# willi-menapace/PlayableVideoGeneration

Hardware: AMD Instinct MI355X
Metric: training clips/sec (B x16x256x256) (higher is better)
Workload: dtype f32; 1 GPU; bair256_t16_b8; variant=main, per_gpu_batch=8, global_batch=8, seq_len=16, gt_init=6, parallelism=dp1

## Files before the change

### include/caddy_hip.h

```cpp
#ifndef CADDY_HIP_H
#define CADDY_HIP_H
#include <stddef.h>
#ifdef __cplusplus
extern "C" {
#endif

typedef struct caddy_ctx caddy_ctx;

typedef struct caddy_config {
    int variant;
    int batch;
    int seq_len;
    int height, width;
    int stacking;
    int actions;
    int action_dim;
    int hidden;
    int use_gumbel, hard_gumbel, use_variations;
    float centroid_alpha;
    int perceptual;
    int ensemble;
} caddy_config;
#define CADDY_MAX_ENSEMBLE 8

// ... 74 lines not shown
int caddy_set_grads_ready_hook(caddy_ctx* ctx, caddy_grads_ready_hook hook, void* user);
int caddy_dp_available(void);
int caddy_dp_unique_id(char* out256);
int caddy_dp_init(caddy_ctx* ctx, const char* id256, int world_size, int rank, int overlap);
int caddy_allreduce_grads(caddy_ctx* ctx);
long caddy_dp_bucket_floats(caddy_ctx* ctx);
int caddy_dp_shutdown(caddy_ctx* ctx);
typedef void (*caddy_sampler_hook)(const float* log_probs, const float* sampled_dirs, float* samples, float* variations,
                                   int n, int K, int Da, int stage, void* user);
int caddy_set_sampler_hook(caddy_ctx* ctx, caddy_sampler_hook hook, void* user, int provides_samples, int provides_variations);
int caddy_set_allreduce_hook(caddy_ctx* ctx, void (*hook)(float* device_ptr, int count, void* user), void* user, int world_size);

int caddy_forward_full(caddy_ctx* ctx, const float* obs, int gt_init, float tau, const caddy_noise* noise, int training,
                       const float* samples_in, const float* variations_in);
int caddy_forward_pretraining(caddy_ctx* ctx, const float* obs, float tau, const caddy_noise* noise, int training,
                              const float* samples_in, const float* variations_in);
int caddy_get_output(caddy_ctx* ctx, int id, void* dst);
int caddy_get_output_grad(caddy_ctx* ctx, int id, void* dst);

int caddy_loss_backward(caddy_ctx* ctx, const caddy_loss_cfg* cfg, double* losses_host);

int caddy_adam_step(caddy_ctx* ctx, float* m, float* v, float lr, float beta1, float beta2, float eps, float weight_decay,
                    int step, float grad_scale);
int caddy_set_action_member(caddy_ctx* ctx, int member);
int caddy_adam_step_member(caddy_ctx* ctx, float* m, float* v, float lr, float beta1, float beta2, float eps, float weight_decay, int step, int member_step, float grad_scale);
int caddy_adam_step_ex(caddy_ctx* ctx, float* m, float* v, float lr, float beta1, float beta2, float eps, float weight_decay, int step, const int* member_step, int s2h_step,
                       float grad_scale);

int caddy_start_inference(caddy_ctx* ctx);
int caddy_f16_saturated(caddy_ctx* ctx);
int caddy_fallback_layers(caddy_ctx* ctx);
int caddy_generate_next(caddy_ctx* ctx, const float* observation, int action, const float* variation, float* frame_out, float* obs_out);

#define CADDY_PROFILE_FAMILIES 18
int caddy_debug_set_poison(caddy_ctx* ctx, int on);
int caddy_debug_set_seeds_only(caddy_ctx* ctx, int on);
int caddy_profile_begin(caddy_ctx* ctx);
int caddy_profile_end(caddy_ctx* ctx, double* out );
int caddy_profile_records(caddy_ctx* ctx, double* out, int max_records);
int caddy_profile_phases(caddy_ctx* ctx, char* names_out, float* ms_out, int max);

int caddy_debug_count(caddy_ctx* ctx);
int caddy_debug_fusion_counts(caddy_ctx* ctx, long* out3);
int caddy_debug_set_bn_paths(caddy_ctx* ctx, int small, int lazy, int epilogue_stats);
int caddy_debug_set_vgg_s16(caddy_ctx* ctx, int on);
int caddy_debug_set_s16_grads(caddy_ctx* ctx, int on);
int caddy_debug_set_perc_chunks(caddy_ctx* ctx, int n);
long caddy_debug_s16_grad_count(caddy_ctx* ctx);
int caddy_debug_set_pack_merged(caddy_ctx* ctx, int on);
int caddy_debug_dims(caddy_ctx* ctx, int i, int* nhwc4);
int caddy_debug_get(caddy_ctx* ctx, int i, int grad, float* dst_nchw);

int caddy_bn_layer_count(caddy_ctx* ctx);
long caddy_bn_calls(caddy_ctx* ctx, int i, char* name_out128);

struct ConvArgs; struct WgradArgs; struct PackDesc; struct TV;
int caddy_k_conv_fwd(const struct ConvArgs* a, void* stream);
int caddy_k_conv_wgrad(const struct WgradArgs* a, void* stream);
int caddy_k_conv_took_direct(void);
int caddy_k_conv_stats_tiles(void);
int caddy_k_bn_finalize_tiles(const float* part, int ntiles, int ldp, long count, const float* gamma, const float* beta, float* rmean, float* rvar, int C,
                              float* mean, float* invstd, float* scale, float* shift, void* stream);
int caddy_k_bn_bwd_lazy(const struct TV* dout, const struct TV* x, const float* mean, const float* invstd, const float* gamma, const float* scale, const float* shift, int act,
                        double* sums, double* scratch, const struct TV* dx, float* dgamma, float* dbeta, void* stream);
int caddy_k_conv_pick_bn(int cout);
int caddy_k_hx_pick_bn(int cout);
int caddy_k_hx_force_big(int v);
// ... 13 lines not shown
```

### playablevideogeneration_amd/csrc/build.py

```python
import os
import subprocess
import sys

HERE = os.path.dirname(os.path.abspath(__file__))
ROOT = os.path.dirname(os.path.dirname(HERE))
SOURCES = ["conv_mfma.hip", "conv_hx.hip", "conv_hx_wgrad.hip", "conv_head.hip", "conv_direct.hip", "conv_thin.hip", "conv_narrow.hip", "conv_stream.hip", "pointwise.hip", "pack.hip", "head.hip", "perceptual.hip", "frame_metrics.hip", "lpips.hip", "detection.hip", "net.cpp", "capi_kernels.cpp", "dp_rccl.cpp"]
LIB = os.path.join(HERE, "libcaddy_hip.so")


def _stale(target, deps):
    if not os.path.exists(target):
        return True
    t = os.path.getmtime(target)
    return any(os.path.getmtime(d) > t for d in deps)


def _deps():
    return [os.path.join(HERE, f) for f in os.listdir(HERE) if f.endswith((".hip", ".cpp", ".h"))] + \
           [os.path.join(ROOT, "include", "caddy_hip.h")]


def _compile_objects(cmd_prefix, objdir, srcs, headers):
    os.makedirs(objdir, exist_ok=True)
    objs, procs = [], []
    for src in srcs:
        obj = os.path.join(objdir, os.path.basename(src) + ".o")
        objs.append(obj)
        if _stale(obj, [src] + headers):
            procs.append((src, subprocess.Popen(cmd_prefix + ["-c", src, "-o", obj])))
    for src, p in procs:
        if p.wait() != 0:
            raise RuntimeError("compile failed: " + src)
    return objs


def build(force=False):
    srcs = [os.path.join(HERE, s) for s in SOURCES if os.path.exists(os.path.join(HERE, s))]
    headers = [d for d in _deps() if d.endswith(".h")]
    if not force and not _stale(LIB, _deps()):
# ... 12 lines not shown
```

### playablevideogeneration_amd/csrc/capi_kernels.cpp

```cpp
#include "common.h"
#include "pointwise.h"
#include "pack.h"

#define ST(s) ((hipStream_t)(s))
extern "C" {
int caddy_k_conv_fwd(const ConvArgs* a, void* s) { return conv_fwd_launch(*a, ST(s)); }
int caddy_k_conv_took_direct(void) { return g_last_conv_direct; }
int caddy_k_conv_stats_tiles(void) { return g_last_conv_stats_tiles; }
int caddy_k_bn_finalize_tiles(const float* part, int ntiles, int ldp, long count, const float* gamma, const float* beta, float* rmean, float* rvar, int C,
                              float* mean, float* invstd, float* scale, float* shift, void* s) {
    return pw_bn_finalize_tiles(part, ntiles, ldp, count, gamma, beta, rmean, rvar, C, mean, invstd, scale, shift, ST(s));
}
int caddy_k_bn_bwd_lazy(const TV* dout, const TV* x, const float* mean, const float* invstd, const float* gamma, const float* scale, const float* shift, int act,
                        double* sums, double* scratch, const TV* dx, float* dgamma, float* dbeta, void* s) {
    int rc = pw_bn_bwd_reduce(*dout, nullptr, *x, mean, invstd, sums, scratch, dgamma, dbeta, ST(s), act ? scale : nullptr, shift);
    return rc ? rc : pw_bn_bwd_apply(*dout, nullptr, *x, mean, invstd, gamma, sums, *dx, nullptr, nullptr, 1, ST(s), act ? scale : nullptr, shift);
}
int caddy_k_conv_wgrad(const WgradArgs* a, void* s) { return conv_wgrad_launch(*a, ST(s)); }
int caddy_k_conv_pick_bn(int cout) { return conv_pick_bn(cout); }
int caddy_k_conv_avgpool_ok(const ConvArgs* a) { return conv_avgpool_ok(*a); }
int caddy_k_hx_pick_bn(int cout) { return hx_pick_bn(cout); }
int caddy_k_hx_force_big(int v) { g_hx_big_override = v; return 0; }
int caddy_k_hx_set_bg(int mask) { g_hx_bg = mask; return 0; }
long caddy_k_hx_weight_bytes(const PackDesc* d, int seg, int rows_pad, int planes) { return (long)hx_weight_bytes(*d, seg, rows_pad, planes); }
int caddy_k_pack_hx(const PackDesc* d, void* wq, int rows_pad, int seg, int precision, void* s) { return pack_hx(*d, wq, rows_pad, seg, precision, ST(s)); }
int caddy_k_pack_fwd(const PackDesc* d, float* wp, void* s) { return pack_fwd(*d, wp, ST(s)); }
int caddy_k_pack_dgrad(const PackDesc* d, int seg, float* wpd, int Cd_pad, int Kd, void* s) { return pack_dgrad(*d, seg, wpd, Cd_pad, Kd, ST(s)); }
int caddy_k_unpack_wgrad(const PackDesc* d, const float* dwp, void* s) { return unpack_wgrad(*d, dwp, ST(s)); }
int caddy_k_adam(float* p, const float* g, float* m, float* v, long n, float lr, float b1, float b2, float eps, float wd, int step, float gscale, void* s) {
    return adam_launch(p, g, m, v, n, lr, b1, b2, eps, wd, step, gscale, ST(s));
}
int caddy_k_copy(const TV* a, const TV* b, int acc, void* s) { return pw_copy(*a, *b, acc, ST(s)); }
int caddy_k_pool2(const TV* in, const TV* out, void* s) { return pw_pool2(*in, *out, ST(s)); }
int caddy_k_pool2_bwd(const TV* dout, const TV* din, void* s) { return pw_pool2_bwd(*dout, *din, 0, ST(s)); }
int caddy_k_up2(const TV* in, const TV* out, void* s) { return pw_up2(*in, *out, ST(s)); }
int caddy_k_up2_bwd(const TV* dout, const TV* din, void* s) { return pw_up2_bwd(*dout, *din, ST(s)); }
int caddy_k_stats(const TV* x, double* sums, void* s) { return pw_stats(*x, sums, nullptr, ST(s)); }
int caddy_k_stats_partials(const TV* x, double* sums, double* scratch, void* s) { return pw_stats(*x, sums, scratch, ST(s)); }
int caddy_k_bn_finalize(const double* sums, long count, const float* gamma, const float* beta, float* rmean, float* rvar, int C, int training,
                        float* mean, float* invstd, float* scale, float* shift, void* s) {
// ... 50 lines not shown
```

### playablevideogeneration_amd/csrc/common.h

```cpp
#pragma once
#include <hip/hip_runtime.h>
#include <cstdint>

typedef float f32x16 __attribute__((ext_vector_type(16)));
typedef float f32x4 __attribute__((ext_vector_type(4)));
typedef __bf16 bf16x8 __attribute__((ext_vector_type(8)));
typedef __bf16 bf16x4 __attribute__((ext_vector_type(4)));

struct TV {
    float* p;
    int N, H, W, C;
    long sn;
    int ld;
    int s16;
};

static inline int cdiv(long a, long b) { return (int)((a + b - 1) / b); }
static inline int round_up(int a, int b) { return (a + b - 1) / b * b; }

#define CONV_MAX_SRC 3
#define CONV_BK 16
struct ConvSrc {
    const float* p;
    long sn;
// ... 60 lines not shown
extern thread_local int g_last_conv_lstm_fused;
#define HX_WSCALE 64.0f
enum { PREC_FP32 = 0, PREC_F16X3 = 16, PREC_BF16X3 = 17, PREC_F16X1 = 18, PREC_BF16X1 = 19 };
#define HX_KC 32
constexpr int CONV_AUX_BYTES = 128 * 1024;

struct WgradArgs {
    ConvSrc src[CONV_MAX_SRC];
    int nsrc;
    int N, H, W;
    int KS;
    const float* dy;
    long dy_sn;
    int dy_ld;
    int Cout, Cout_pad;
    int Ktot;
    float* dwp;
    int slabs;
    int group_n;
    long src_gs[CONV_MAX_SRC];
    long dy_gs;
    int precision;
    long src_bn_gs[CONV_MAX_SRC];
    float* det_slab;
    long det_cap;
    long det_stride;
    int dy_s16;
};
#define WGRAD_DST(a_, split_) ((a_).det_slab ? (a_).det_slab + (long)(split_) * (a_).det_stride : (a_).dwp)
long wgrad_det_begin(WgradArgs& a, long splits, hipStream_t st);
int wgrad_det_end(const WgradArgs& a, long splits, hipStream_t st);

enum { CK_FWD_128x128 = 0, CK_FWD_128x64, CK_FWD_64x64, CK_FWD_128x32, CK_THIN_OUT, CK_THIN_IN, CK_WGRAD_128, CK_WGRAD_64, CK_WGRAD_32, CK_WGRAD_SMALL, CK_WGRAD_THIN, CK_WGRAD_TILE, CK_NARROW,
       CK_HX_128, CK_HX_64, CK_HX_32, CK_WGRAD_HX, CK_HX_128_8W, CK_COUNT };
extern thread_local int g_last_conv_kernel;
static inline long conv_stats_tiles_cap(int N, int H, int W) { long t = (long)N * cdiv(H, 8) * cdiv(W, 16); return t > 512 ? t : 512; }
extern thread_local int g_last_conv_stats_tiles;
extern thread_local int g_last_conv_direct;
bool conv_src_lazy_ok(const ConvArgs& a);
bool wgrad_src_lazy_ok(const WgradArgs& a);
int conv_fwd_launch(const ConvArgs& a, hipStream_t st);
int conv_wgrad_launch(const WgradArgs& a, hipStream_t st);
int conv_pick_bn(int cout);
struct PackDesc;
int conv_hx_wgrad_try(const WgradArgs& a, hipStream_t st, bool dry = false);
int conv_hx_try(const ConvArgs& a, hipStream_t st, bool dry = false);
bool conv_hx_s16_ok(int N, int H, int W, int Cout);
bool conv_hx_pool_ok(int N, int H, int W, int Cout);
int pack_hx(const PackDesc& d, void* wq, int rows_pad, int seg , int precision, hipStream_t st);
size_t hx_weight_bytes(const PackDesc& d, int seg, int rows_pad, int planes);
int hx_kq(const PackDesc& d, int seg);
int hx_pick_bn(int cout);
template <int NPL> __host__ __device__ __forceinline__ long hx_wq_piece(int row, int g) { return ((long)((row >> 5) * 2 + (g >> 1)) * NPL) * 64 + (g & 1) * 32 + (row & 31); }
extern int g_hx_big_override;
extern int g_hx_bg;
int conv_split_reduce_pool_launch(const float* scr, long stride, int splits, int ldc, int N, int H, int W, int C, float* out, long out_sn, int out_ld, const float* bias, int act,
                                  const float* res, long res_sn, int res_ld, hipStream_t st);
int conv_split_reduce_lstm_launch(const float* scr, long stride, int splits, int ldc, int HW, long P, const float* bias, const LstmFuse& f, hipStream_t st);
int conv_split_reduce_launch(const float* scr, long stride, int splits, int ldc, int HW, long P, int C, float* out, long out_sn, int out_ld, const float* bias, int act,
                             const float* res, long res_sn, int res_ld, hipStream_t st, float* stats = nullptr, int stats_ld = 0, long stats_cap_tiles = 0, int accumulate = 0);
int conv_thin_fwd_try(const ConvArgs& a, hipStream_t st);
int conv_head_fwd_try(const ConvArgs& a, hipStream_t st);
int conv_head_dgrad_try(const ConvArgs& a, hipStream_t st);
int conv_hx_avgpool_ok(const ConvArgs& a);
int conv1x1_lat_try(const ConvArgs& a, hipStream_t st, bool dry = false);
int conv_direct_try(const ConvArgs& a, hipStream_t st, bool dry = false);
int conv_stream_wgrad_try(const WgradArgs& a, hipStream_t st, bool dry = false);
int conv_head_wgrad_try(const WgradArgs& a, hipStream_t st, bool dry = false);
extern thread_local int g_last_wgrad_grouped;
int conv_narrow_wgrad_try(const WgradArgs& a, hipStream_t st, bool dry = false);
int conv_c4_wgrad_try(const WgradArgs& a, hipStream_t st, bool dry = false);
int conv_c4_fwd_try(const ConvArgs& a, hipStream_t st);
int conv_narrow_fwd_try(const ConvArgs& a, hipStream_t st);
int conv_narrow_fwd_ok(const ConvArgs& a);
int conv_thin_wgrad_try(const WgradArgs& a, hipStream_t st, bool dry = false);
```

### playablevideogeneration_amd/csrc/conv_mfma.hip

```cpp
#include "common.h"
#include <cstdlib>

namespace {

constexpr int BK = CONV_BK;
constexpr int LDSK = BK + 4;

struct SegRef { const float* p; long sn; int ld; int C; int bcast; int c0; int idx; };

__device__ __forceinline__ SegRef find_seg(const ConvSrc* src, int nsrc, int k) {
    int s = 0;
    while (s + 1 < nsrc && k >= src[s].Cpad) { k -= src[s].Cpad; s++; }
    SegRef r; r.p = src[s].p; r.sn = src[s].sn; r.ld = src[s].ld; r.C = src[s].C; r.bcast = src[s].bcast; r.c0 = k; r.idx = s;
    return r;
}

__device__ __forceinline__ float4 load4_masked(const float* q, int c, int C) {
    float4 v = make_float4(0.f, 0.f, 0.f, 0.f);
    if (c + 4 <= C) v = *reinterpret_cast<const float4*>(q);
    else {
        if (c < C) v.x = q[0];
        if (c + 1 < C) v.y = q[1];
        if (c + 2 < C) v.z = q[2];
    }
// ... 857 lines not shown
    const long blocks = cdiv(a.det_stride, 256);
    hipLaunchKernelGGL(k_wgrad_det_reduce, dim3((unsigned)(blocks > 2048 ? 2048 : blocks)), dim3(256), 0, st, a.dwp, (const float*)a.det_slab, (int)splits, a.det_stride);
    return 0;
}

static int conv_wgrad_launch1(const WgradArgs& a0, hipStream_t st, bool dry);
int conv_wgrad_launch(const WgradArgs& a0, hipStream_t st) {
    if (a0.group_n <= 0 || a0.N <= a0.group_n) return conv_wgrad_launch1(a0, st, false);
    if (conv_wgrad_launch1(a0, st, true) == 0 && (g_last_conv_kernel == CK_WGRAD_TILE || g_last_conv_kernel == CK_WGRAD_HX || g_last_wgrad_grouped)) return conv_wgrad_launch1(a0, st, false);
    for (int g = 0; g * a0.group_n < a0.N; g++) {
        WgradArgs a = a0;
        a.N = a0.group_n; a.group_n = 0;
        for (int s = 0; s < a0.nsrc; s++) a.src[s].p = a0.src[s].p + g * a0.src_gs[s];
        a.dy = a0.dy + g * a0.dy_gs;
        int rc = conv_wgrad_launch1(a, st, false);
        if (rc) return rc;
    }
    return 0;
}
static int conv_wgrad_launch1(const WgradArgs& a0, hipStream_t st, bool dry) {
    WgradArgs a = a0;
    if (a.nsrc < 1 || a.nsrc > CONV_MAX_SRC) return -1;
    int bn = conv_pick_bn(a.Cout);
    if (a.Cout_pad != round_up(a.Cout, bn)) return -1;
    if (a.group_n > 0 && a.N <= a.group_n) a.group_n = 0;
    if (conv_hx_wgrad_try(a, st, dry) == 1) return 0;
    if (a.dy_s16) return -1;
    for (int s = 0; s < a.nsrc; s++) if (a.src[s].bn_scale) return -1;
    g_last_wgrad_grouped = 0;
    { int rc = conv_stream_wgrad_try(a, st, dry); if (rc != 0) return rc < 0 ? rc : 0; }
    { int rc = conv_head_wgrad_try(a, st, dry); if (rc != 0) return rc < 0 ? rc : 0; }
    if (conv_c4_wgrad_try(a, st, dry) == 1) return 0;
    if (conv_thin_wgrad_try(a, st, dry) == 1) return 0;
    if (conv_narrow_wgrad_try(a, st, dry) == 1) return 0;
    long P = (long)a.N * a.H * a.W;
    int taps = a.KS * a.KS;
    if (a.nsrc == 1 && !a.src[0].bcast && a.Cout <= 32 && a.Ktot <= 64 && a.KS <= 3 && P >= 4096 && !(a.Ktot > 32 && a.KS == 3)) {
        int tx = cdiv(a.W, STW), ty = cdiv(a.H, STH);
        long ntiles = (long)a.N * tx * ty;
        int grid = (int)(ntiles < 512 ? ntiles : 512);
        g_last_conv_kernel = CK_WGRAD_SMALL;
        if (dry) return 0;
        if (a.det_slab) { grid = (int)wgrad_det_begin(a, grid, st); if (grid <= 0) return -1; }
        if (a.Ktot <= 32) hipLaunchKernelGGL((k_conv_wgrad_small<1>), dim3(grid), dim3(256), 0, st, a, tx, ty);
        else hipLaunchKernelGGL((k_conv_wgrad_small<2>), dim3(grid), dim3(256), 0, st, a, tx, ty);
        if (a.det_slab) wgrad_det_end(a, grid, st);
        g_last_conv_kernel = CK_WGRAD_SMALL;
        return 0;
    }
    if (a.KS == 3 && a.W >= 8 && a.H >= 2) {
        int tx = cdiv(a.W, WT_W), ty = cdiv(a.H, WT_H);
        long ntiles = (long)a.N * tx * ty;
        int kt = cdiv(a.Ktot, WT_KC);
        bool o32 = a.Cout <= 32;
        int ot = o32 ? 1 : cdiv(a.Cout, 64);
        const int tile_blocks = 256;
        long g = tile_blocks / ((long)kt * ot);
        if (g < 1) g = 1;
        if (g > ntiles) g = ntiles;
        g_last_conv_kernel = CK_WGRAD_TILE;
        if (dry) return 0;
        if (a.det_slab) { g = wgrad_det_begin(a, g, st); if (g <= 0) return -1; }
        dim3 grid(kt, ot, (unsigned)g);
        if (o32) hipLaunchKernelGGL((k_conv_wgrad_tile<1>), grid, dim3(256), 0, st, a, tx, ty);
        else hipLaunchKernelGGL((k_conv_wgrad_tile<2>), grid, dim3(256), 0, st, a, tx, ty);
        if (a.det_slab) wgrad_det_end(a, g, st);
        g_last_conv_kernel = CK_WGRAD_TILE;
// ... 26 lines not shown
```

### playablevideogeneration_amd/csrc/conv_narrow.hip

```cpp
#include "common.h"
#include <cstdlib>

namespace {
constexpr int NTW = 32, NTH = 8, NHW = NTW + 2, NHH = NTH + 2;
typedef float f32x4 __attribute__((ext_vector_type(4)));

__device__ __forceinline__ float4 nld4(const float* q, int c, int C) {
    float4 v = make_float4(0.f, 0.f, 0.f, 0.f);
    if (c + 4 <= C) v = *reinterpret_cast<const float4*>(q);
    else { if (c < C) v.x = q[0]; if (c + 1 < C) v.y = q[1]; if (c + 2 < C) v.z = q[2]; }
    return v;
}

template <int CI4, int NT>
__global__ __launch_bounds__(256) void k_conv_narrow(ConvArgs a, int tiles_x, int tiles_y) {
    constexpr int CI = 16 * CI4, PITCH = CI + 4, Q = CI / 4;
    constexpr int NLOAD = (NHH * NHW * Q + 255) / 256;
    __shared__ float xs[NHH * NHW * PITCH];
    const int tid = threadIdx.x, lane = tid & 63, wave = tid >> 6;
    const int lp = lane & 15, g = lane >> 4;
    const ConvSrc s = a.src[0];
    const long ntiles = (long)a.N * tiles_x * tiles_y;

    float4 w[9][NT][CI4];
// ... 117 lines not shown

static bool narrow_shape_ok(const ConvArgs& a) {
    if (a.nsrc != 1 || a.src[0].bcast || a.src[0].bn_scale || a.KS != 3 || (a.act != 0 && a.act != 3) || a.splitk > 1) return false;
    if (a.Ktot > 32 || a.Cout > 32 || a.src[0].C <= 4 || a.Cout <= 4) return false;
    if (a.src[0].C <= 12 && a.Cout < 16) return false;
    if ((a.src[0].ld & 3) || (a.src[0].sn & 3) || a.Cout_pad < 16 * ((a.Cout + 15) / 16)) return false;
    if (a.mask || a.pool_out || a.skip_out || a.in_s16 || a.out_s16) return false;
    if ((long)a.N * a.H * a.W < 4096) return false;
    if (a.avgpool && ((a.H | a.W) & 1)) return false;
    return true;
}
int conv_narrow_fwd_ok(const ConvArgs& a) { return narrow_shape_ok(a) ? 1 : 0; }
int conv_avgpool_ok(const ConvArgs& a) {
    if (a.wq && a.precision >= PREC_F16X3) return conv_hx_avgpool_ok(a);
    ConvArgs b = a; b.avgpool = 1; b.splitk = 1;
    if (a.KS == 1) return conv1x1_lat_try(b, nullptr, true);
    return narrow_shape_ok(b) ? 1 : 0;
}

int conv_narrow_fwd_try(const ConvArgs& a, hipStream_t st) {
    if (!narrow_shape_ok(a) || (a.out_ld & 3) || (a.out_sn & 3)) return 0;
    const int tx = cdiv(a.W, NTW), ty = cdiv(a.H, NTH);
    const long ntiles = (long)a.N * tx * ty;
    const int grid = (int)(ntiles < 1024 ? ntiles : 1024);
    const int ci4 = a.Ktot / 16, nt = (a.Cout + 15) / 16;
    if (ci4 == 1 && nt == 1) hipLaunchKernelGGL((k_conv_narrow<1, 1>), dim3(grid), dim3(256), 0, st, a, tx, ty);
    else if (ci4 == 1) hipLaunchKernelGGL((k_conv_narrow<1, 2>), dim3(grid), dim3(256), 0, st, a, tx, ty);
    else if (nt == 1) hipLaunchKernelGGL((k_conv_narrow<2, 1>), dim3(grid), dim3(256), 0, st, a, tx, ty);
    else hipLaunchKernelGGL((k_conv_narrow<2, 2>), dim3(grid), dim3(256), 0, st, a, tx, ty);
    g_last_conv_kernel = CK_NARROW;
    return 1;
}

namespace {
template <int CI16, int CO16>
__global__ __launch_bounds__(256) void k_wgrad_narrow(WgradArgs a, int tiles_x, int tiles_y) {
    constexpr int PX = CI16 == 1 ? 16 : 48, PY = CO16 == 1 ? 16 : 48;
    constexpr int QX = 4 * CI16, QY = 4 * CO16;
    constexpr int NX = (NHH * NHW * QX + 255) / 256, NY = NTH * NTW * QY / 256;
    __shared__ float xs[NHH * NHW * PX];
    __shared__ float ys[NTH * NTW * PY];
    const int tid = threadIdx.x, lane = tid & 63, wave = tid >> 6;
    const int lp = lane & 15, g = lane >> 4;
    const ConvSrc s = a.src[0];
    const long ntiles = (long)a.N * tiles_x * tiles_y;
    f32x4 acc[9][CO16][CI16];
#pragma unroll
    for (int t = 0; t < 9; t++)
#pragma unroll
        for (int m = 0; m < CO16; m++)
#pragma unroll
            for (int n = 0; n < CI16; n++) acc[t][m][n] = f32x4{0.f, 0.f, 0.f, 0.f};

    float4 px[NX], py[NY];
    auto gload = [&](long tile) {
        int n = (int)(tile / (tiles_x * tiles_y));
        int rem = (int)(tile - (long)n * tiles_x * tiles_y);
        int ty = rem / tiles_x;
        int y0 = ty * NTH, x0 = (rem - ty * tiles_x) * NTW;
        const float* bx = s.p + (long)n * s.sn;
        const float* by = a.dy + (long)n * a.dy_sn;
#pragma unroll
        for (int i = 0; i < NX; i++) {
            int idx = tid + 256 * i, hp = idx / QX, c = (idx % QX) * 4;
            int hy = hp / NHW, hx = hp - hy * NHW;
            int y = y0 - 1 + hy, x = x0 - 1 + hx;
            px[i] = make_float4(0.f, 0.f, 0.f, 0.f);
            if (hp < NHH * NHW && y >= 0 && y < a.H && x >= 0 && x < a.W && c < s.C) px[i] = nld4(bx + ((long)y * a.W + x) * s.ld + c, c, s.C);
        }
#pragma unroll
        for (int i = 0; i < NY; i++) {
            int idx = tid + 256 * i, p = idx / QY, c = (idx % QY) * 4;
            int y = y0 + p / NTW, x = x0 + (p & (NTW - 1));
            py[i] = make_float4(0.f, 0.f, 0.f, 0.f);
            if (y < a.H && x < a.W && c < a.Cout) py[i] = nld4(by + ((long)y * a.W + x) * a.dy_ld + c, c, a.Cout);
        }
    };

    long tile = blockIdx.x;
    if (tile < ntiles) gload(tile);
    for (; tile < ntiles; tile += gridDim.x) {
#pragma unroll
        for (int i = 0; i < NX; i++) {
            int idx = tid + 256 * i, hp = idx / QX;
            if (hp < NHH * NHW) *reinterpret_cast<float4*>(&xs[hp * PX + (idx % QX) * 4]) = px[i];
        }
#pragma unroll
        for (int i = 0; i < NY; i++) {
            int idx = tid + 256 * i;
            *reinterpret_cast<float4*>(&ys[(idx / QY) * PY + (idx % QY) * 4]) = py[i];
        }
        __syncthreads();
        if (tile + gridDim.x < ntiles) gload(tile + gridDim.x);
#pragma unroll 2
        for (int grp = 0; grp < 16; grp++) {
            const int row = 2 * wave + (grp >> 3), x0 = 4 * (grp & 7) + g;
            float fa[CO16];
#pragma unroll
            for (int m = 0; m < CO16; m++) fa[m] = ys[(row * NTW + x0) * PY + m * 16 + lp];
#pragma unroll
            for (int t = 0; t < 9; t++) {
                const int dy = t / 3, dx = t - 3 * dy;
                const float* xp = &xs[((row + dy) * NHW + x0 + dx) * PX + lp];
#pragma unroll
                for (int n = 0; n < CI16; n++) {
                    const float fb = xp[n * 16];
#pragma unroll
                    for (int m = 0; m < CO16; m++) acc[t][m][n] = __builtin_amdgcn_mfma_f32_16x16x4f32(fa[m], fb, acc[t][m][n], 0, 0, 0);
                }
            }
        }
        __syncthreads();
    }
    constexpr int NW = 9 * CO16 * 16 * CI16 * 16;
    static_assert(NW <= NHH * NHW * PX, "LDS reduction buffer must fit in the X tile");
    float* red = xs;
    for (int i = tid; i < NW; i += 256) red[i] = 0.f;
    __syncthreads();
    for (int wv = 0; wv < 4; wv++) {
        if (wave == wv) {
#pragma unroll
            for (int t = 0; t < 9; t++)
#pragma unroll
                for (int m = 0; m < CO16; m++)
#pragma unroll
                    for (int n = 0; n < CI16; n++)
#pragma unroll
                        for (int r = 0; r < 4; r++) red[((t * CO16 * 16) + m * 16 + 4 * g + r) * (CI16 * 16) + n * 16 + lp] += acc[t][m][n][r];
        }
        __syncthreads();
    }
    float* const dst = WGRAD_DST(a, blockIdx.x);
    for (int i = tid; i < NW; i += 256) {
        int k = i % (CI16 * 16), to = i / (CI16 * 16);
        int o = to % (CO16 * 16), t = to / (CO16 * 16);
        if (k < a.Ktot && o < a.Cout) atomicAdd(dst + ((long)t * a.Cout_pad + o) * a.Ktot + k, red[i]);
    }
}
}

int conv_narrow_wgrad_try(const WgradArgs& a, hipStream_t st, bool dry) {
    if (a.nsrc != 1 || a.src[0].bcast || a.KS != 3) return 0;
    if (a.Ktot > 32 || a.Cout > 32 || a.src[0].C <= 12 || a.Cout <= 4) return 0;
    const int ci = a.Ktot / 16, co = (a.Cout + 15) / 16;
    if (ci == 2 && co == 2) return 0;
    if ((a.src[0].ld & 3) || (a.src[0].sn & 3) || (a.dy_ld & 3) || (a.dy_sn & 3)) return 0;
    if ((long)a.N * a.H * a.W < 4096) return 0;
    const int tx = cdiv(a.W, NTW), ty = cdiv(a.H, NTH);
    const long ntiles = (long)a.N * tx * ty;
    long want = ntiles / 4;
    const int grid = (int)(want < 64 ? (ntiles < 64 ? ntiles : 64) : (want < 512 ? want : 512));
    g_last_conv_kernel = CK_WGRAD_SMALL;
    if (dry) return 1;
    WgradArgs b = a;
    int gridn = grid;
    if (b.det_slab) { gridn = (int)wgrad_det_begin(b, grid, st); if (gridn <= 0) return -1; }
    if (ci == 1 && co == 1) hipLaunchKernelGGL((k_wgrad_narrow<1, 1>), dim3(gridn), dim3(256), 0, st, b, tx, ty);
    else if (ci == 1) hipLaunchKernelGGL((k_wgrad_narrow<1, 2>), dim3(gridn), dim3(256), 0, st, b, tx, ty);
    else hipLaunchKernelGGL((k_wgrad_narrow<2, 1>), dim3(gridn), dim3(256), 0, st, b, tx, ty);
    if (b.det_slab) wgrad_det_end(b, gridn, st);
    g_last_conv_kernel = CK_WGRAD_SMALL;
    return 1;
}

namespace {
template <int KS, int NT>
__global__ __launch_bounds__(256) void k_conv_c4(ConvArgs a, int tiles_x, int tiles_y) {
    constexpr int R = KS / 2, HW_ = NTW + 2 * R, HH_ = NTH + 2 * R, TAPS = KS * KS;
    constexpr int NL = (HH_ * HW_ + 255) / 256;
    __shared__ float xs[HH_ * HW_ * 4];
    const int tid = threadIdx.x, lane = tid & 63, wave = tid >> 6;
    const int lp = lane & 15, g = lane >> 4;
    const ConvSrc s = a.src[0];
    const long ntiles = (long)a.N * tiles_x * tiles_y;
    const int og = blockIdx.y * NT * 16;

    __shared__ float ws[TAPS * NT * 64];
    for (int i = tid; i < TAPS * NT * 64; i += 256) {
        int l = i & 63, tm = i >> 6;
        int m = tm % NT, t = tm / NT;
        ws[i] = a.wp[((long)t * a.Cout_pad + og + m * 16 + (l & 15)) * a.Ktot + (l >> 4)];
    }
    float4 pre[NL];
    auto gload = [&](long tile) {
        int n = (int)(tile / (tiles_x * tiles_y));
        int rem = (int)(tile - (long)n * tiles_x * tiles_y);
        int ty = rem / tiles_x;
        int y0 = ty * NTH, x0 = (rem - ty * tiles_x) * NTW;
        const float* base = s.p + (long)n * s.sn;
#pragma unroll
        for (int i = 0; i < NL; i++) {
            int hp = tid + 256 * i;
            int hy = hp / HW_, hx = hp - hy * HW_;
            int y = y0 - R + hy, x = x0 - R + hx;
            pre[i] = make_float4(0.f, 0.f, 0.f, 0.f);
            if (hp < HH_ * HW_ && y >= 0 && y < a.H && x >= 0 && x < a.W) pre[i] = nld4(base + ((long)y * a.W + x) * 4, 0, s.C);
// ... 210 lines not shown
```

### playablevideogeneration_amd/engine.py

```python
import ctypes as C
import os
from typing import Dict, List, Optional

import torch

from . import _lib

LOSS_NAMES = ["total", "rec", "states", "entropy", "dir_kl", "mi", "state_kl", "hidden", "l1_r0", "l1_r1", "l1_r2", "perceptual", "perceptual_term"]
LOSS_SLOTS, LOSS_PERC_R0, DIAG_0 = 56, 16, 40
DIAG_NAMES = ["samples_entropy", "action_distribution_entropy", "states_magnitude", "hidden_states_magnitude", "action_directions_mean_magnitude",
              "action_directions_variance_magnitude", "reconstructed_action_directions_mean_magnitude", "reconstructed_action_directions_variance_magnitude",
              "action_directions_reconstruction_error", "reconstructed_action_directions_kl_loss", "centroids_mean_magnitude", "average_centroids_distance",
              "average_action_variations_norm_l2", "action_variations_mean"]


class CaddyConfig(C.Structure):
    _fields_ = [("variant", C.c_int), ("batch", C.c_int), ("seq_len", C.c_int), ("height", C.c_int), ("width", C.c_int),
                ("stacking", C.c_int), ("actions", C.c_int), ("action_dim", C.c_int), ("hidden", C.c_int),
                ("use_gumbel", C.c_int), ("hard_gumbel", C.c_int), ("use_variations", C.c_int), ("centroid_alpha", C.c_float),
                ("perceptual", C.c_int), ("ensemble", C.c_int)]


class ParamInfo(C.Structure):
    _fields_ = [("name", C.c_char * 128), ("offset", C.c_long), ("ndim", C.c_int), ("shape", C.c_int * 4), ("kind", C.c_int)]
# ... 458 lines not shown
        out = torch.zeros(5, self.B, Trec, dtype=torch.float64)
        self._stream()
        self._check(self.lib.caddy_perceptual_per_frame(self.ctx, out.data_ptr()))
        return out

    def numerics_flags(self) -> int:
        return int(self.lib.caddy_f16_saturated(self.ctx))

    def f16_saturated(self) -> bool:
        return bool(self.numerics_flags() & 1)

    def fallback_layers(self) -> int:
        return int(self.lib.caddy_fallback_layers(self.ctx))

    def start_inference(self):
        self._stream()
        self._check(self.lib.caddy_start_inference(self.ctx))

    def generate_next(self, observation: torch.Tensor, action: int, variation: Optional[torch.Tensor] = None):
        S, H, W = self.S, self.H, self.W
        obs = observation.to(self.device, torch.float32).contiguous()
        assert tuple(obs.shape) == (3 * S, H, W)
        frame = torch.empty((3, H, W), dtype=torch.float32, device=self.device)
        nxt = torch.empty((3 * S, H, W), dtype=torch.float32, device=self.device)
        v = variation.to(self.device, torch.float32).contiguous() if variation is not None else None
        self._stream()
        self._check(self.lib.caddy_generate_next(self.ctx, obs.data_ptr(), int(action), v.data_ptr() if v is not None else None,
                                                 frame.data_ptr(), nxt.data_ptr()))
        return frame, nxt

    CONV_FAMILIES = ["k_conv_fwd<2, 2, 2, 2, 0, 1>", "k_conv_fwd<2, 1, 2, 2, 0, 1>", "k_conv_fwd<1, 1, 2, 2, 0, 1>", "k_conv_fwd<1, 1, 4, 1, 0, 1>",
                     "k_conv_thin_out", "k_conv_thin_in", "k_conv_wgrad<2, 2, 2, 2>", "k_conv_wgrad<1, 2, 2, 2>", "k_conv_wgrad<1, 1, 1, 4>",
                     "k_conv_wgrad_small", "k_wgrad_thin", "k_conv_wgrad_tile", "k_conv_narrow",
                     "k_conv_hx<128>", "k_conv_hx<64>", "k_conv_hx<32>", "k_wgrad_hx", "k_conv_hx<128, 8 waves>"]

    def profile_begin(self):
        self._check(self.lib.caddy_profile_begin(C.c_void_p(self.ctx)))

    def profile_records(self, max_records=20000):
        buf = (C.c_double * (7 * max_records))()
        n = self.lib.caddy_profile_records(C.c_void_p(self.ctx), buf, max_records)
        return [tuple(buf[7 * i + j] for j in range(7)) for i in range(n)]

    def profile_phases(self, max_marks=256):
        names = C.create_string_buffer(48 * max_marks)
        ms = (C.c_float * max_marks)()
        n = self.lib.caddy_profile_phases(C.c_void_p(self.ctx), names, ms, max_marks)
        return [(names.raw[48 * i:48 * (i + 1)].split(b"\0")[0].decode(), ms[i]) for i in range(n)]

    def profile_end(self):
        out = (C.c_double * (4 * len(self.CONV_FAMILIES)))()
        self._check(self.lib.caddy_profile_end(C.c_void_p(self.ctx), out))
        return {n: (int(out[4 * i]), out[4 * i + 1], out[4 * i + 2], out[4 * i + 3]) for i, n in enumerate(self.CONV_FAMILIES)}

    def fusion_counts(self) -> Dict[str, int]:
        out = (C.c_long * 3)()
        self.lib.caddy_debug_fusion_counts(C.c_void_p(self.ctx), out)
        return {"bn_calls": out[0], "stats_from_conv_epilogue": out[1], "never_materialised": out[2]}

    def bn_calls(self) -> Dict[str, int]:
        buf = C.create_string_buffer(128)
        res = {}
        for i in range(self.lib.caddy_bn_layer_count(self.ctx)):
            n = self.lib.caddy_bn_calls(self.ctx, i, buf)
            res[buf.value.decode()] = n
        return res
```

Before: 65.35 clips/s.

## Replace narrow wgrad kernel with row-tiled pixel-pair MFMA wgrad

Replaces the narrow 3x3 weight-gradient kernel with a new row-tiled kernel. It stores pixel pairs interleaved in shared memory so each X load is reused across horizontal taps. Each block works on a contiguous run of tiles sized from the CU count, and a deterministic slab path writes per-block partials that a separate fold kernel sums. It also covers the 2x2 channel-block case the old kernel skipped and supports grouped batches. In exchange it adds a second kernel launch in deterministic mode and uses more registers for the double-buffered loads.

```diff
diff --git a/include/caddy_hip.h b/include/caddy_hip.h
--- a/include/caddy_hip.h
+++ b/include/caddy_hip.h
@@ -130,7 +130,7 @@
 int caddy_fallback_layers(caddy_ctx* ctx);
 int caddy_generate_next(caddy_ctx* ctx, const float* observation, int action, const float* variation, float* frame_out, float* obs_out);
 
-#define CADDY_PROFILE_FAMILIES 18
+#define CADDY_PROFILE_FAMILIES 19
 int caddy_debug_set_poison(caddy_ctx* ctx, int on);
 int caddy_debug_set_seeds_only(caddy_ctx* ctx, int on);
 int caddy_profile_begin(caddy_ctx* ctx);
diff --git a/playablevideogeneration_amd/csrc/build.py b/playablevideogeneration_amd/csrc/build.py
--- a/playablevideogeneration_amd/csrc/build.py
+++ b/playablevideogeneration_amd/csrc/build.py
@@ -4,7 +4,7 @@
 
 HERE = os.path.dirname(os.path.abspath(__file__))
 ROOT = os.path.dirname(os.path.dirname(HERE))
-SOURCES = ["conv_mfma.hip", "conv_hx.hip", "conv_hx_wgrad.hip", "conv_head.hip", "conv_direct.hip", "conv_thin.hip", "conv_narrow.hip", "conv_stream.hip", "pointwise.hip", "pack.hip", "head.hip", "perceptual.hip", "frame_metrics.hip", "lpips.hip", "detection.hip", "net.cpp", "capi_kernels.cpp", "dp_rccl.cpp"]
+SOURCES = ["conv_mfma.hip", "conv_hx.hip", "conv_hx_wgrad.hip", "conv_head.hip", "conv_direct.hip", "conv_thin.hip", "conv_narrow.hip", "conv_wgrad_rows.hip", "conv_stream.hip", "pointwise.hip", "pack.hip", "head.hip", "perceptual.hip", "frame_metrics.hip", "lpips.hip", "detection.hip", "net.cpp", "capi_kernels.cpp", "dp_rccl.cpp"]
 LIB = os.path.join(HERE, "libcaddy_hip.so")
 
 
diff --git a/playablevideogeneration_amd/csrc/capi_kernels.cpp b/playablevideogeneration_amd/csrc/capi_kernels.cpp
--- a/playablevideogeneration_amd/csrc/capi_kernels.cpp
+++ b/playablevideogeneration_amd/csrc/capi_kernels.cpp
@@ -6,6 +6,7 @@
 extern "C" {
 int caddy_k_conv_fwd(const ConvArgs* a, void* s) { return conv_fwd_launch(*a, ST(s)); }
 int caddy_k_conv_took_direct(void) { return g_last_conv_direct; }
+int caddy_k_conv_last_kernel(void) { return g_last_conv_kernel; }
 int caddy_k_conv_stats_tiles(void) { return g_last_conv_stats_tiles; }
 int caddy_k_bn_finalize_tiles(const float* part, int ntiles, int ldp, long count, const float* gamma, const float* beta, float* rmean, float* rvar, int C,
                               float* mean, float* invstd, float* scale, float* shift, void* s) {
diff --git a/playablevideogeneration_amd/csrc/common.h b/playablevideogeneration_amd/csrc/common.h
--- a/playablevideogeneration_amd/csrc/common.h
+++ b/playablevideogeneration_amd/csrc/common.h
@@ -116,7 +116,7 @@
 int wgrad_det_end(const WgradArgs& a, long splits, hipStream_t st);
 
 enum { CK_FWD_128x128 = 0, CK_FWD_128x64, CK_FWD_64x64, CK_FWD_128x32, CK_THIN_OUT, CK_THIN_IN, CK_WGRAD_128, CK_WGRAD_64, CK_WGRAD_32, CK_WGRAD_SMALL, CK_WGRAD_THIN, CK_WGRAD_TILE, CK_NARROW,
-       CK_HX_128, CK_HX_64, CK_HX_32, CK_WGRAD_HX, CK_HX_128_8W, CK_COUNT };
+       CK_HX_128, CK_HX_64, CK_HX_32, CK_WGRAD_HX, CK_HX_128_8W, CK_WGRAD_ROWS, CK_COUNT };
 extern thread_local int g_last_conv_kernel;
 static inline long conv_stats_tiles_cap(int N, int H, int W) { long t = (long)N * cdiv(H, 8) * cdiv(W, 16); return t > 512 ? t : 512; }
 extern thread_local int g_last_conv_stats_tiles;
@@ -152,7 +152,7 @@
 int conv_stream_wgrad_try(const WgradArgs& a, hipStream_t st, bool dry = false);
 int conv_head_wgrad_try(const WgradArgs& a, hipStream_t st, bool dry = false);
 extern thread_local int g_last_wgrad_grouped;
-int conv_narrow_wgrad_try(const WgradArgs& a, hipStream_t st, bool dry = false);
+int conv_wgrad_rows_try(const WgradArgs& a, hipStream_t st, bool dry = false);
 int conv_c4_wgrad_try(const WgradArgs& a, hipStream_t st, bool dry = false);
 int conv_c4_fwd_try(const ConvArgs& a, hipStream_t st);
 int conv_narrow_fwd_try(const ConvArgs& a, hipStream_t st);
diff --git a/playablevideogeneration_amd/csrc/conv_mfma.hip b/playablevideogeneration_amd/csrc/conv_mfma.hip
--- a/playablevideogeneration_amd/csrc/conv_mfma.hip
+++ b/playablevideogeneration_amd/csrc/conv_mfma.hip
@@ -913,7 +913,7 @@
     { int rc = conv_head_wgrad_try(a, st, dry); if (rc != 0) return rc < 0 ? rc : 0; }
     if (conv_c4_wgrad_try(a, st, dry) == 1) return 0;
     if (conv_thin_wgrad_try(a, st, dry) == 1) return 0;
-    if (conv_narrow_wgrad_try(a, st, dry) == 1) return 0;
+    { int rc = conv_wgrad_rows_try(a, st, dry); if (rc != 0) return rc < 0 ? rc : 0; }
     long P = (long)a.N * a.H * a.W;
     int taps = a.KS * a.KS;
     if (a.nsrc == 1 && !a.src[0].bcast && a.Cout <= 32 && a.Ktot <= 64 && a.KS <= 3 && P >= 4096 && !(a.Ktot > 32 && a.KS == 3)) {
diff --git a/playablevideogeneration_amd/csrc/conv_narrow.hip b/playablevideogeneration_amd/csrc/conv_narrow.hip
--- a/playablevideogeneration_amd/csrc/conv_narrow.hip
+++ b/playablevideogeneration_amd/csrc/conv_narrow.hip
@@ -173,136 +173,6 @@
     return 1;
 }
 
-namespace {
-template <int CI16, int CO16>
-__global__ __launch_bounds__(256) void k_wgrad_narrow(WgradArgs a, int tiles_x, int tiles_y) {
-    constexpr int PX = CI16 == 1 ? 16 : 48, PY = CO16 == 1 ? 16 : 48;
-    constexpr int QX = 4 * CI16, QY = 4 * CO16;
-    constexpr int NX = (NHH * NHW * QX + 255) / 256, NY = NTH * NTW * QY / 256;
-    __shared__ float xs[NHH * NHW * PX];
-    __shared__ float ys[NTH * NTW * PY];
-    const int tid = threadIdx.x, lane = tid & 63, wave = tid >> 6;
-    const int lp = lane & 15, g = lane >> 4;
-    const ConvSrc s = a.src[0];
-    const long ntiles = (long)a.N * tiles_x * tiles_y;
-    f32x4 acc[9][CO16][CI16];
-#pragma unroll
-    for (int t = 0; t < 9; t++)
-#pragma unroll
-        for (int m = 0; m < CO16; m++)
-#pragma unroll
-            for (int n = 0; n < CI16; n++) acc[t][m][n] = f32x4{0.f, 0.f, 0.f, 0.f};
-
-    float4 px[NX], py[NY];
-    auto gload = [&](long tile) {
-        int n = (int)(tile / (tiles_x * tiles_y));
-        int rem = (int)(tile - (long)n * tiles_x * tiles_y);
-        int ty = rem / tiles_x;
-        int y0 = ty * NTH, x0 = (rem - ty * tiles_x) * NTW;
-        const float* bx = s.p + (long)n * s.sn;
-        const float* by = a.dy + (long)n * a.dy_sn;
-#pragma unroll
-        for (int i = 0; i < NX; i++) {
-            int idx = tid + 256 * i, hp = idx / QX, c = (idx % QX) * 4;
-            int hy = hp / NHW, hx = hp - hy * NHW;
-            int y = y0 - 1 + hy, x = x0 - 1 + hx;
-            px[i] = make_float4(0.f, 0.f, 0.f, 0.f);
-            if (hp < NHH * NHW && y >= 0 && y < a.H && x >= 0 && x < a.W && c < s.C) px[i] = nld4(bx + ((long)y * a.W + x) * s.ld + c, c, s.C);
-        }
-#pragma unroll
-        for (int i = 0; i < NY; i++) {
-            int idx = tid + 256 * i, p = idx / QY, c = (idx % QY) * 4;
-            int y = y0 + p / NTW, x = x0 + (p & (NTW - 1));
-            py[i] = make_float4(0.f, 0.f, 0.f, 0.f);
-            if (y < a.H && x < a.W && c < a.Cout) py[i] = nld4(by + ((long)y * a.W + x) * a.dy_ld + c, c, a.Cout);
-        }
-    };
-
-    long tile = blockIdx.x;
-    if (tile < ntiles) gload(tile);
-    for (; tile < ntiles; tile += gridDim.x) {
-#pragma unroll
-        for (int i = 0; i < NX; i++) {
-            int idx = tid + 256 * i, hp = idx / QX;
-            if (hp < NHH * NHW) *reinterpret_cast<float4*>(&xs[hp * PX + (idx % QX) * 4]) = px[i];
-        }
-#pragma unroll
-        for (int i = 0; i < NY; i++) {
-            int idx = tid + 256 * i;
-            *reinterpret_cast<float4*>(&ys[(idx / QY) * PY + (idx % QY) * 4]) = py[i];
-        }
-        __syncthreads();
-        if (tile + gridDim.x < ntiles) gload(tile + gridDim.x);
-#pragma unroll 2
-        for (int grp = 0; grp < 16; grp++) {
-            const int row = 2 * wave + (grp >> 3), x0 = 4 * (grp & 7) + g;
-            float fa[CO16];
-#pragma unroll
-            for (int m = 0; m < CO16; m++) fa[m] = ys[(row * NTW + x0) * PY + m * 16 + lp];
-#pragma unroll
-            for (int t = 0; t < 9; t++) {
-                const int dy = t / 3, dx = t - 3 * dy;
-                const float* xp = &xs[((row + dy) * NHW + x0 + dx) * PX + lp];
-#pragma unroll
-                for (int n = 0; n < CI16; n++) {
-                    const float fb = xp[n * 16];
-#pragma unroll
-                    for (int m = 0; m < CO16; m++) acc[t][m][n] = __builtin_amdgcn_mfma_f32_16x16x4f32(fa[m], fb, acc[t][m][n], 0, 0, 0);
-                }
-            }
-        }
-        __syncthreads();
-    }
-    constexpr int NW = 9 * CO16 * 16 * CI16 * 16;
-    static_assert(NW <= NHH * NHW * PX, "LDS reduction buffer must fit in the X tile");
-    float* red = xs;
-    for (int i = tid; i < NW; i += 256) red[i] = 0.f;
-    __syncthreads();
-    for (int wv = 0; wv < 4; wv++) {
-        if (wave == wv) {
-#pragma unroll
-            for (int t = 0; t < 9; t++)
-#pragma unroll
-                for (int m = 0; m < CO16; m++)
-#pragma unroll
-                    for (int n = 0; n < CI16; n++)
-#pragma unroll
-                        for (int r = 0; r < 4; r++) red[((t * CO16 * 16) + m * 16 + 4 * g + r) * (CI16 * 16) + n * 16 + lp] += acc[t][m][n][r];
-        }
-        __syncthreads();
-    }
-    float* const dst = WGRAD_DST(a, blockIdx.x);
-    for (int i = tid; i < NW; i += 256) {
-        int k = i % (CI16 * 16), to = i / (CI16 * 16);
-        int o = to % (CO16 * 16), t = to / (CO16 * 16);
-        if (k < a.Ktot && o < a.Cout) atomicAdd(dst + ((long)t * a.Cout_pad + o) * a.Ktot + k, red[i]);
-    }
-}
-}
-
-int conv_narrow_wgrad_try(const WgradArgs& a, hipStream_t st, bool dry) {
-    if (a.nsrc != 1 || a.src[0].bcast || a.KS != 3) return 0;
-    if (a.Ktot > 32 || a.Cout > 32 || a.src[0].C <= 12 || a.Cout <= 4) return 0;
-    const int ci = a.Ktot / 16, co = (a.Cout + 15) / 16;
-    if (ci == 2 && co == 2) return 0;
-    if ((a.src[0].ld & 3) || (a.src[0].sn & 3) || (a.dy_ld & 3) || (a.dy_sn & 3)) return 0;
-    if ((long)a.N * a.H * a.W < 4096) return 0;
-    const int tx = cdiv(a.W, NTW), ty = cdiv(a.H, NTH);
-    const long ntiles = (long)a.N * tx * ty;
-    long want = ntiles / 4;
-    const int grid = (int)(want < 64 ? (ntiles < 64 ? ntiles : 64) : (want < 512 ? want : 512));
-    g_last_conv_kernel = CK_WGRAD_SMALL;
-    if (dry) return 1;
-    WgradArgs b = a;
-    int gridn = grid;
-    if (b.det_slab) { gridn = (int)wgrad_det_begin(b, grid, st); if (gridn <= 0) return -1; }
-    if (ci == 1 && co == 1) hipLaunchKernelGGL((k_wgrad_narrow<1, 1>), dim3(gridn), dim3(256), 0, st, b, tx, ty);
-    else if (ci == 1) hipLaunchKernelGGL((k_wgrad_narrow<1, 2>), dim3(gridn), dim3(256), 0, st, b, tx, ty);
-    else hipLaunchKernelGGL((k_wgrad_narrow<2, 1>), dim3(gridn), dim3(256), 0, st, b, tx, ty);
-    if (b.det_slab) wgrad_det_end(b, gridn, st);
-    g_last_conv_kernel = CK_WGRAD_SMALL;
-    return 1;
-}
 
 namespace {
 template <int KS, int NT>
diff --git a/playablevideogeneration_amd/csrc/conv_wgrad_rows.hip b/playablevideogeneration_amd/csrc/conv_wgrad_rows.hip
--- /dev/null
+++ b/playablevideogeneration_amd/csrc/conv_wgrad_rows.hip
@@ -0,0 +1,232 @@
+#include "common.h"
+
+namespace {
+constexpr int RW_TH = 8;
+
+__device__ __forceinline__ float4 rw_ld4(const float* q, int c, int C) {
+    float4 v = make_float4(0.f, 0.f, 0.f, 0.f);
+    if (c + 4 <= C) v = *reinterpret_cast<const float4*>(q);
+    else { if (c < C) v.x = q[0]; if (c + 1 < C) v.y = q[1]; if (c + 2 < C) v.z = q[2]; }
+    return v;
+}
+
+template <int CI16, int CO16, int TW>
+__global__ __launch_bounds__(256) void k_wgrad_rows(WgradArgs a, int tiles_x, int tiles_y, int tpw) {
+    constexpr int CI = 16 * CI16, CO = 16 * CO16;
+    constexpr int PPX = CI16 == 1 ? 32 : 96, PPY = CO16 == 1 ? 32 : 96;
+    constexpr int HWP = TW / 2 + 1, HH = RW_TH + 2, TWP = TW / 2;
+    constexpr int QX = CI / 4, QY = CO / 4;
+    constexpr int NIX = HH * HWP * QX, NIY = RW_TH * TWP * QY;
+    constexpr int NX = (NIX + 255) / 256, NY = NIY / 256;
+    constexpr int GR = TW / 8;
+    static_assert(NIY % 256 == 0, "dY items must divide evenly");
+    __shared__ __attribute__((aligned(16))) float xs[HH * HWP * PPX];
+    __shared__ __attribute__((aligned(16))) float ys[RW_TH * TWP * PPY];
+    const int tid = threadIdx.x, lane = tid & 63, wave = tid >> 6;
+    const int lp = lane & 15, g = lane >> 4;
+    const ConvSrc s = a.src[0];
+    const long ntiles = (long)a.N * tiles_x * tiles_y;
+    const long t_beg = (long)blockIdx.x * tpw, t_end = t_beg + tpw < ntiles ? t_beg + tpw : ntiles;
+    f32x4 acc[9][CO16][CI16];
+#pragma unroll
+    for (int t = 0; t < 9; t++)
+#pragma unroll
+        for (int m = 0; m < CO16; m++)
+#pragma unroll
+            for (int n = 0; n < CI16; n++) acc[t][m][n] = f32x4{0.f, 0.f, 0.f, 0.f};
+
+    float4 xa[NX], xb[NX], ya[NY], yb[NY];
+    auto gload = [&](long tile) {
+        int n = (int)(tile / (tiles_x * tiles_y));
+        const int rem = (int)(tile - (long)n * tiles_x * tiles_y);
+        const int ty = rem / tiles_x;
+        const int y0 = ty * RW_TH, x0 = (rem - ty * tiles_x) * TW;
+        const float* bx = s.p;
+        const float* by = a.dy;
+        if (a.group_n > 0) { const int grp = n / a.group_n; n -= grp * a.group_n; bx += grp * a.src_gs[0]; by += grp * a.dy_gs; }
+        bx += (long)n * s.sn; by += (long)n * a.dy_sn;
+#pragma unroll
+        for (int i = 0; i < NX; i++) {
+            const int idx = tid + 256 * i, hp = idx / QX, c = (idx % QX) * 4;
+            const int hy = hp / HWP, hq = hp - hy * HWP;
+            const int y = y0 - 1 + hy, x = x0 - 1 + 2 * hq;
+            xa[i] = make_float4(0.f, 0.f, 0.f, 0.f); xb[i] = xa[i];
+            if (idx < NIX && y >= 0 && y < a.H && c < s.C) {
+                const float* q = bx + ((long)y * a.W + x) * s.ld + c;
+                if (x >= 0 && x < a.W) xa[i] = rw_ld4(q, c, s.C);
+                if (x + 1 < a.W) xb[i] = rw_ld4(q + s.ld, c, s.C);
+            }
+        }
+#pragma unroll
+        for (int i = 0; i < NY; i++) {
+            const int idx = tid + 256 * i, p2 = idx / QY, c = (idx % QY) * 4;
+            const int row = p2 / TWP, q2 = p2 - row * TWP;
+            const int y = y0 + row, x = x0 + 2 * q2;
+            ya[i] = make_float4(0.f, 0.f, 0.f, 0.f); yb[i] = ya[i];
+            if (y < a.H && c < a.Cout) {
+                const float* q = by + ((long)y * a.W + x) * a.dy_ld + c;
+                if (x < a.W) ya[i] = rw_ld4(q, c, a.Cout);
+                if (x + 1 < a.W) yb[i] = rw_ld4(q + a.dy_ld, c, a.Cout);
+            }
+        }
+    };
+
+    long tile = t_beg;
+    if (tile < t_end) gload(tile);
+    for (; tile < t_end; tile++) {
+#pragma unroll
+        for (int i = 0; i < NX; i++) {
+            const int idx = tid + 256 * i, hp = idx / QX, c = (idx % QX) * 4;
+            if (idx < NIX) {
+                float* d = &xs[hp * PPX + 2 * c];
+                *reinterpret_cast<float4*>(d) = make_float4(xa[i].x, xb[i].x, xa[i].y, xb[i].y);
+                *reinterpret_cast<float4*>(d + 4) = make_float4(xa[i].z, xb[i].z, xa[i].w, xb[i].w);
+            }
+        }
+#pragma unroll
+        for (int i = 0; i < NY; i++) {
+            const int idx = tid + 256 * i, p2 = idx / QY, c = (idx % QY) * 4;
+            float* d = &ys[p2 * PPY + 2 * c];
+            *reinterpret_cast<float4*>(d) = make_float4(ya[i].x, yb[i].x, ya[i].y, yb[i].y);
+            *reinterpret_cast<float4*>(d + 4) = make_float4(ya[i].z, yb[i].z, ya[i].w, yb[i].w);
+        }
+        __syncthreads();
+        if (tile + 1 < t_end) gload(tile + 1);
+#pragma unroll 2
+        for (int grp = 0; grp < 2 * GR; grp++) {
+            const int row = 2 * wave + grp / GR, q0 = 4 * (grp % GR) + g;
+            float2 fa[CO16];
+#pragma unroll
+            for (int m = 0; m < CO16; m++) fa[m] = *reinterpret_cast<const float2*>(&ys[(row * TWP + q0) * PPY + 2 * (m * 16 + lp)]);
+#pragma unroll
+            for (int dy = 0; dy < 3; dy++) {
+                const float* xp = &xs[((row + dy) * HWP + q0) * PPX + 2 * lp];
+                float fb[CI16][4];
+#pragma unroll
+                for (int n = 0; n < CI16; n++) {
+                    const float2 r0 = *reinterpret_cast<const float2*>(xp + 32 * n), r1 = *reinterpret_cast<const float2*>(xp + PPX + 32 * n);
+                    fb[n][0] = r0.x; fb[n][1] = r0.y; fb[n][2] = r1.x; fb[n][3] = r1.y;
+                }
+#pragma unroll
+                for (int e = 0; e < 2; e++)
+#pragma unroll
+                    for (int dx = 0; dx < 3; dx++)
+#pragma unroll
+                        for (int m = 0; m < CO16; m++)
+#pragma unroll
+                            for (int n = 0; n < CI16; n++)
+                                acc[dy * 3 + dx][m][n] = __builtin_amdgcn_mfma_f32_16x16x4f32(e ? fa[m].y : fa[m].x, fb[n][e + dx], acc[dy * 3 + dx][m][n], 0, 0, 0);
+            }
+        }
+        __syncthreads();
+    }
+    constexpr int NW = 9 * CO * CI;
+    static_assert(NW <= HH * HWP * PPX, "fold buffer must fit in the X image");
+    float* red = xs;
+    for (int wv = 0; wv < 4; wv++) {
+        if (wave == wv) {
+#pragma unroll
+            for (int t = 0; t < 9; t++)
+#pragma unroll
+                for (int m = 0; m < CO16; m++)
+#pragma unroll
+                    for (int n = 0; n < CI16; n++)
+#pragma unroll
+                        for (int r = 0; r < 4; r++) {
+                            float* d = &red[((t * CO) + m * 16 + 4 * g + r) * CI + n * 16 + lp];
+                            *d = wv == 0 ? acc[t][m][n][r] : *d + acc[t][m][n][r];
+                        }
+        }
+        __syncthreads();
+    }
+    float* const dst = WGRAD_DST(a, blockIdx.x);
+    if (a.det_slab) {
+        for (long i = 4 * tid; i < a.det_stride; i += 1024) {
+            const int k = (int)(i % a.Ktot);
+            const long to = i / a.Ktot;
+            const int o = (int)(to % a.Cout_pad), t = (int)(to / a.Cout_pad);
+            float4 v = make_float4(0.f, 0.f, 0.f, 0.f);
+            if (t < 9 && o < CO && k < CI) v = *reinterpret_cast<const float4*>(&red[(t * CO + o) * CI + k]);
+            *reinterpret_cast<float4*>(dst + i) = v;
+        }
+    } else {
+        for (int i = tid; i < NW; i += 256) {
+            const int k = i % CI, to = i / CI;
+            const int o = to % CO, t = to / CO;
+            if (k < a.Ktot && o < a.Cout) atomicAdd(dst + ((long)t * a.Cout_pad + o) * a.Ktot + k, red[i]);
+        }
+    }
+}
+
+__global__ __launch_bounds__(256) void k_wgrad_rows_fold(float* dwp, const float* slab, int splits, long stride) {
+    __shared__ float sh[3][64];
+    const int lane = threadIdx.x & 63, w = threadIdx.x >> 6;
+    const long i = (long)blockIdx.x * 64 + lane;
+    float v = 0.f;
+    if (i < stride) {
+        int s = w;
+        for (; s + 28 < splits; s += 32) {
+            float u[8];
+#pragma unroll
+            for (int j = 0; j < 8; j++) u[j] = slab[(long)(s + 4 * j) * stride + i];
+#pragma unroll
+            for (int j = 0; j < 8; j++) v += u[j];
+        }
+        for (; s < splits; s += 4) v += slab[(long)s * stride + i];
+    }
+    if (w > 0) sh[w - 1][lane] = v;
+    __syncthreads();
+    if (w == 0 && i < stride) {
+        v += sh[0][lane]; v += sh[1][lane]; v += sh[2][lane];
+        dwp[i] += v;
+    }
+}
+
+int rw_cu_count() {
+    static int cus = 0;
+    if (cus <= 0) {
+        cus = 256;
+#if defined(__HIPCC__)
+        int dev = 0, n = 0;
+        if (hipGetDevice(&dev) == hipSuccess && hipDeviceGetAttribute(&n, hipDeviceAttributeMultiprocessorCount, dev) == hipSuccess && n > 0) cus = n;
+#endif
+    }
+    return cus;
+}
+}
+
+int conv_wgrad_rows_try(const WgradArgs& a0, hipStream_t st, bool dry) {
+    if (a0.nsrc != 1 || a0.src[0].bcast || a0.src[0].bn_scale || a0.dy_s16 || a0.KS != 3) return 0;
+    if (a0.src[0].C <= 12 || a0.src[0].C > 32 || a0.Cout <= 4 || a0.Cout > 32 || a0.Ktot != round_up(a0.src[0].C, CONV_BK)) return 0;
+    if ((a0.src[0].ld & 3) || (a0.src[0].sn & 3) || (a0.dy_ld & 3) || (a0.dy_sn & 3) || a0.Cout_pad < a0.Cout) return 0;
+    if (a0.group_n > 0 && a0.N > a0.group_n && ((a0.src_gs[0] & 3) || (a0.dy_gs & 3))) return 0;
+    if ((long)a0.N * a0.H * a0.W < 4096) return 0;
+    const int ci = a0.Ktot / 16, co = (a0.Cout + 15) / 16;
+    const int TW = (ci == 1 && co == 1) ? 64 : 32;
+    const int tx = cdiv(a0.W, TW), ty = cdiv(a0.H, RW_TH);
+    const long ntiles = (long)a0.N * tx * ty;
+    if (ntiles >= (1L << 30)) return 0;
+    g_last_conv_kernel = CK_WGRAD_ROWS;
+    g_last_wgrad_grouped = 1;
+    if (dry) return 1;
+    WgradArgs a = a0;
+    if (a.group_n > 0 && a.N <= a.group_n) a.group_n = 0;
+    long want = (long)rw_cu_count() * (TW == 64 ? 2 : 1);
+    if (a.det_slab) {
+        a.det_stride = ((long)9 * a.Cout_pad * a.Ktot + 3) / 4 * 4;
+        const long fit = a.det_cap / a.det_stride;
+        if (fit < 1) return -1;
+        if (want > fit) want = fit;
+    }
+    if (want > ntiles) want = ntiles;
+    const int tpw = cdiv(ntiles, want);
+    const int grid = cdiv(ntiles, tpw);
+#define RW_LAUNCH(CI_, CO_, TW_) hipLaunchKernelGGL((k_wgrad_rows<CI_, CO_, TW_>), dim3(grid), dim3(256), 0, st, a, tx, ty, tpw)
+    if (ci == 1 && co == 1) RW_LAUNCH(1, 1, 64);
+    else if (ci == 1) RW_LAUNCH(1, 2, 32);
+    else if (co == 1) RW_LAUNCH(2, 1, 32);
+    else RW_LAUNCH(2, 2, 32);
+#undef RW_LAUNCH
+    if (a.det_slab) hipLaunchKernelGGL(k_wgrad_rows_fold, dim3(cdiv(a.det_stride, 64)), dim3(256), 0, st, a.dwp, (const float*)a.det_slab, grid, a.det_stride);
+    return 1;
+}
diff --git a/playablevideogeneration_amd/engine.py b/playablevideogeneration_amd/engine.py
--- a/playablevideogeneration_amd/engine.py
+++ b/playablevideogeneration_amd/engine.py
@@ -514,7 +514,7 @@
     CONV_FAMILIES = ["k_conv_fwd<2, 2, 2, 2, 0, 1>", "k_conv_fwd<2, 1, 2, 2, 0, 1>", "k_conv_fwd<1, 1, 2, 2, 0, 1>", "k_conv_fwd<1, 1, 4, 1, 0, 1>",
                      "k_conv_thin_out", "k_conv_thin_in", "k_conv_wgrad<2, 2, 2, 2>", "k_conv_wgrad<1, 2, 2, 2>", "k_conv_wgrad<1, 1, 1, 4>",
                      "k_conv_wgrad_small", "k_wgrad_thin", "k_conv_wgrad_tile", "k_conv_narrow",
-                     "k_conv_hx<128>", "k_conv_hx<64>", "k_conv_hx<32>", "k_wgrad_hx", "k_conv_hx<128, 8 waves>"]
+                     "k_conv_hx<128>", "k_conv_hx<64>", "k_conv_hx<32>", "k_wgrad_hx", "k_conv_hx<128, 8 waves>", "k_wgrad_rows"]
 
     def profile_begin(self):
         self._check(self.lib.caddy_profile_begin(C.c_void_p(self.ctx)))
```

After: 65.65 clips/s (median of 6 runs). About the same (+0.5%).
